# KrishnaswamyLab/MELD

Measured on AMD Instinct MI355X. Metric: cells/sec through MELD.fit_transform (kNN+Chebyshev), higher is better.
Workload: dtype f64

## Files before the change

include/meld_hip.h:

```cpp
#ifndef MELD_HIP_H
#define MELD_HIP_H

#include <stddef.h>
#include <stdint.h>

#ifdef __cplusplus
extern "C" {
#endif

#define MELD_OK 0
#define MELD_ERR_INVALID (-1)
#define MELD_ERR_UNSUPPORTED (-2)
#define MELD_ERR_HIP (-3)

typedef void* meld_stream_t;

int meld_abi_version(void);
const char* meld_last_error(void);
int meld_device_count(void);


int meld_knn_padded_dim(int d);
int meld_knn_tile_refs(void);
int meld_knn_block_queries(void);
// ... 50 lines not shown
                      int nprod, void* temp, void* lb2, meld_stream_t stream);
int meld_knn16_prepare_cross(const double* X, int64_t n_refs, int64_t n_total, int d, const double* mean, int64_t q_begin,
                             int64_t q_count, void* Rt16, void* Q16, float* Qn, float* norm2, float* norm2_max,
                             float* scale_info, meld_stream_t stream);
int meld_knn16_prepare_rows(const double* X, int64_t N, int d, const double* mean, const float* scale_info,
                            int64_t q_begin, const int32_t* rows, int64_t n_rows, void* Q16, float* Qn,
                            meld_stream_t stream);
int meld_knn16_research_thresholds(const int32_t* rows, int64_t n_rows, int64_t q_begin, const int32_t* cand_cnt,
                                   const float* cand_d2, int cap, int ksel, const float* norm2, const float* norm2_max,
                                   double err_coef, double err_lin, double err3, const float* scale_info, float* thr,
                                   meld_stream_t stream);
int meld_knn16_seed_thresholds_mfma(const void* Q16, const float* Qn, const void* Rt16, const float* scale_info,
                                    const float* norm2_max, int64_t n_ref, int d, int64_t q_begin, int64_t q_count,
                                    int knn, double radius_factor, int nprod, int side_tiles, float* thr_init,
                                    meld_stream_t stream);
int meld_knn16_topk(const void* Q16, const float* Qn, const void* Rt16, const float* scale_info,
                    int64_t n_ref, int d, int64_t q_count, int ksel, int nprod, int n_slices, const void* lb2,
                    const float* norm2_max, int64_t q_begin, const float* thr_init, int knn, double radius_factor,
                    int32_t* cand_idx, float* cand_d2, int32_t* cand_cnt, float* cand_thr,
                    uint64_t* tiles_done ,
                    const int32_t* block_order ,
                    meld_stream_t stream);
int meld_knn16_block_work(const void* lb2, const float* thr_seed, int64_t n_ref, int d, int64_t q_count, int nprod,
                          const float* norm2_max, const float* scale_info, int32_t* work, meld_stream_t stream);
int meld_knn16_step_lists(const void* lb2, const float* thr_seed, int64_t n_ref, int d, int64_t q_count, int nprod,
                          const float* norm2_max, const float* scale_info, int64_t q_begin, uint32_t* list,
                          int64_t list_stride, int32_t* cnt, meld_stream_t stream);
size_t meld_knn16_list_scratch_bytes(int64_t n_ref);
int meld_knn16_step_lists_direct(const double* X, int64_t N, int d, const double* mean, const float* scale_info, const float* norm2_max,
                                 const void* Rt16, const float* thr_seed, const float* q_norm2, int nprod, void* temp, void* scratch,
                                 uint32_t* list, int64_t list_stride, int32_t* cnt, meld_stream_t stream);
int meld_knn16_step_lists_direct_lead(const double* X, int64_t N, int d, const double* mean, const float* scale_info, const float* norm2_max,
                                 const void* Rt16, const float* thr_seed, const float* q_norm2, int nprod, void* temp, void* scratch,
                                 uint32_t* list, int64_t list_stride, int32_t* cnt, int lead_only, meld_stream_t stream);
int meld_knn16_step_lists_direct_spheres(const double* X, int64_t N, int d, const double* mean, const float* scale_info, const float* norm2_max,
                                 const void* Rt16, const float* thr_seed, const float* q_norm2, int nprod, void* temp, void* scratch,
                                 uint32_t* list, int64_t list_stride, int32_t* cnt, int lead_only, meld_stream_t stream);
int meld_knn16_topk_listed(const void* Q16, const float* Qn, const void* Rt16, const float* scale_info, int64_t n_ref, int d,
                           int64_t q_count, int ksel, const uint32_t* step_list, const int32_t* step_cnt, int64_t list_stride,
                           const float* norm2_max, int64_t q_begin, const float* thr_init, int knn, double radius_factor,
                           int32_t* cand_idx, float* cand_d2, int32_t* cand_cnt, float* cand_thr, uint64_t* tiles_done,
                           const int32_t* block_order, int n_slices , meld_stream_t stream);
int meld_knn16_topk_listed_partial(const void* Q16, const float* Qn, const void* Rt16, const float* scale_info, int64_t n_ref,
                                   int d, int64_t q_count, int ksel, const uint32_t* step_list, const int32_t* step_cnt,
                                   int64_t list_stride, const float* norm2_max, int64_t q_begin, const float* thr_init, int knn,
                                   double radius_factor, int32_t* cand_idx, float* cand_d2, int32_t* cand_cnt, float* cand_thr,
                                   uint64_t* tiles_done, const int32_t* block_order, int n_slices, int partial_test,
                                   meld_stream_t stream);
int meld_knn16_partial_filter(const void* Q16, const float* Qn, const void* Rt16, const float* scale_info, const float* norm2_max, int d,
                              int64_t q_count, const float* thr_init, uint32_t* step_list, const int32_t* step_cnt, int64_t list_stride,
                              int32_t* cnt_out, uint64_t* tested, const int32_t* block_order , meld_stream_t stream);
int meld_knn16_resident_blocks(int d, int nprod);
int meld_knn16_max_slices(int ksel);
int meld_knn16_merge_slices(const int32_t* s_idx, const float* s_d2, const int32_t* s_cnt, int64_t q_count,
                            int ksel, int n_slices, int32_t* out_idx, float* out_d2, int32_t* out_cnt,
                            meld_stream_t stream);


int meld_knn_refine(const double* X, int64_t N, int d, int64_t q_begin, int64_t q_count,
                    const int32_t* cand_idx, const float* cand_d2, const int32_t* cand_cnt,
                    const float* cand_thr ,
                    int ksel, int cap , int knn, double decay, double thresh,
                    const float* norm2_max, double err_coef,
                    const float* norm2 , double err_coef_lin, double* bw,
                    double* cand_val, int32_t* keep_cnt, int32_t* flag_rows, int32_t* n_flag,
                    const int32_t* rows, int out_cap, int32_t* cand_idx_out,
                    double bw_scale ,
                    const double* bw_fixed ,
                    int max_rank ,
                    meld_stream_t stream);

int meld_knn_radius_exact(const double* X, int64_t N, int d, int64_t q_begin, const int32_t* flag_rows,
                          int32_t n_flag, const double* bw, int knn, double decay, double thresh,
                          int mode, int32_t* fb_cnt, const int64_t* fb_off, int32_t* fb_cursor,
                          int32_t* fb_col, double* fb_val, int32_t* err_flag,
                          double bw_scale ,
                          meld_stream_t stream);
int meld_knn_pair_distances(const double* X, int d, const int64_t* rows, const int64_t* cand, int64_t n, int kk, double* out,
                            meld_stream_t stream);

#define MELD_METRIC_L1 1
#define MELD_METRIC_LINF 2
int meld_metric_tile_rows(void);
int meld_metric_tile_boxes(const double* X, int64_t N, int d, double* box_lo, double* box_hi, meld_stream_t stream);
int meld_metric_topk(const double* X, int64_t N, int d, int metric, int ksel, const double* box_lo, const double* box_hi, int prune,
                     double* heap_d, int32_t* heap_i, int32_t* cand_idx, double* cand_d, int32_t* cand_cnt,
                     unsigned long long* tiles_done, meld_stream_t stream);
int meld_metric_refine(const int32_t* cand_idx, const double* cand_d, const int32_t* cand_cnt, int64_t N, int ksel, int knn,
                       double decay, double thresh, double* bw, double* cand_val, int32_t* keep_cnt, int32_t* flag_rows,
                       int32_t* n_flag, meld_stream_t stream);
int meld_metric_radius(const double* X, int64_t N, int d, int metric, const int32_t* flag_rows, int32_t n_flag, const double* bw,
                       double decay, double thresh, int mode, int32_t* fb_cnt, const int64_t* fb_off, int32_t* fb_cursor,
                       int32_t* fb_col, double* fb_val, meld_stream_t stream);


size_t meld_scan_temp_bytes(int64_t n);
int meld_exclusive_scan_i32_i64(const int32_t* in, int64_t* out, int64_t n, void* temp, size_t temp_bytes,
                                meld_stream_t stream);

int meld_coo_emit(int64_t q_begin, int64_t q_count, const int32_t* cand_idx, const double* cand_val,
                  const int32_t* cand_cnt, int ksel, int cap, const int64_t* keep_off, const int32_t* flag_rows,
                  int32_t n_flag, const int64_t* fb_off, const int32_t* fb_col, const double* fb_val,
                  int64_t fb_base, int64_t M, uint64_t* keys, double* vals, meld_stream_t stream);

size_t meld_sort_temp_bytes(int64_t n);
int meld_sort_pairs_u64_f64(const uint64_t* keys_in, uint64_t* keys_out, const double* vals_in,
// ... 166 lines not shown
```

meld_amd/_lib.py:

```python
from __future__ import annotations

from ._options import is_set, opt

import ctypes as C
import os

_HERE = os.path.dirname(os.path.abspath(__file__))
LIB_NAME = "libmeld_hip.so"
LIB_PATH = os.path.join(_HERE, LIB_NAME)

_i32, _i64, _f64, _sz, _ptr = C.c_int, C.c_int64, C.c_double, C.c_size_t, C.c_void_p

SIGNATURES = {
    "meld_abi_version": (_i32, []),
    "meld_last_error": (C.c_char_p, []),
    "meld_device_count": (_i32, []),
    "meld_knn_padded_dim": (_i32, [_i32]),
    "meld_knn_tile_refs": (_i32, []),
    "meld_knn_block_queries": (_i32, []),
    "meld_knn_row_capacity": (_i32, [_i32]),
    "meld_col_sums_f64": (_i32, [_ptr, _i64, _i32, _ptr, _ptr]),
    "meld_col_stats_temp_bytes": (_sz, [_i32]),
    "meld_col_stats_f64": (_i32, [_ptr, _i64, _i32, _ptr, _ptr, _ptr, _ptr, _sz, _ptr]),
    "meld_knn_prepare_refs": (_i32, [_ptr, _i64, _i32, _ptr, _i32, _ptr, _ptr, _ptr, _ptr]),
    "meld_knn_prepare_queries": (_i32, [_ptr, _i64, _i32, _ptr, _i32, _i64, _i64, _ptr, _ptr]),
    "meld_knn_topk": (_i32, [_ptr, _ptr, _i64, _i32, _i64, _i32, _ptr, _ptr, _ptr, _ptr]),
    "meld_knn_refine": (
        _i32,
        [_ptr, _i64, _i32, _i64, _i64, _ptr, _ptr, _ptr, _ptr, _i32, _i32, _i32, _f64, _f64, _ptr, _f64, _ptr, _f64, _ptr, _ptr, _ptr,
         _ptr, _ptr, _ptr, _i32, _ptr, _f64, _ptr, _i32, _ptr],
    ),
    "meld_knn_error_coef": (_f64, [_i32]),
    "meld_knn16_kblocks": (_i32, [_i32]),
    "meld_knn16_tile_refs": (_i32, []),
    "meld_knn16_split_dims": (_i32, [_i32]),
    "meld_knn16_block_queries": (_i32, []),
    "meld_knn16_row_capacity": (_i32, [_i32]),
    "meld_knn16_error_coef": (_f64, [_i32, _i32]),
    "meld_knn16_error_coef_const": (_f64, [_i32, _i32]),
    "meld_knn16_error_coef_lin": (_f64, [_i32]),
    "meld_knn16_resident_blocks": (_i32, [_i32, _i32]),
    "meld_knn16_tile_bytes": (_sz, [_i32]),
    "meld_knn16_query_bytes": (_sz, [_i32]),
    "meld_knn16_prepare": (_i32, [_ptr, _i64, _i32, _ptr, _i64, _i64, _ptr, _ptr, _ptr, _ptr, _ptr, _ptr, _ptr]),
    "meld_knn16_prepare_scaled": (_i32, [_ptr, _i64, _i32, _ptr, _ptr, _ptr, _i64, _i64, _ptr, _ptr, _ptr, _ptr, _ptr, _ptr, _ptr]),
    "meld_knn16_prepare_cross": (_i32, [_ptr, _i64, _i64, _i32, _ptr, _i64, _i64, _ptr, _ptr, _ptr, _ptr, _ptr, _ptr, _ptr]),
    "meld_knn16_prepare_rows": (_i32, [_ptr, _i64, _i32, _ptr, _ptr, _i64, _ptr, _i64, _ptr, _ptr, _ptr]),
    "meld_knn16_research_thresholds": (_i32, [_ptr, _i64, _i64, _ptr, _ptr, _i32, _i32, _ptr, _ptr, _f64, _f64, _f64, _ptr, _ptr, _ptr]),
    "meld_knn16_bounds_bytes": (_sz, [_i64, _i64]),
    "meld_knn16_bounds_temp_bytes": (_sz, [_i64, _i32, _i64]),
    "meld_knn16_bounds": (_i32, [_ptr, _i64, _i32, _ptr, _ptr, _ptr, _ptr, _i64, _i64, _ptr, _ptr, _i32, _ptr, _ptr, _ptr]),
    "meld_knn16_bounds_from_spheres": (_i32, [_ptr, _i64, _i32, _ptr, _ptr, _ptr, _ptr, _i64, _i64, _ptr, _ptr, _i32, _ptr, _ptr, _ptr]),
    "meld_knn16_tile_spheres": (_i32, [_ptr, _i64, _i32, _ptr, _ptr, _ptr, _i64, _i64, _ptr]),
    "meld_knn16_sphere_layout": (_i32, [_i64, _i32, _ptr, _ptr]),
    "meld_knn16_topk": (_i32, [_ptr, _ptr, _ptr, _ptr, _i64, _i32, _i64, _i32, _i32, _i32, _ptr, _ptr, _i64, _ptr, _i32, _f64, _ptr, _ptr, _ptr, _ptr, _ptr, _ptr, _ptr]),
    "meld_knn16_block_work": (_i32, [_ptr, _ptr, _i64, _i32, _i64, _i32, _ptr, _ptr, _ptr, _ptr]),
    "meld_knn16_step_lists": (_i32, [_ptr, _ptr, _i64, _i32, _i64, _i32, _ptr, _ptr, _i64, _ptr, _i64, _ptr, _ptr]),
    "meld_knn16_list_scratch_bytes": (_sz, [_i64]),
    "meld_knn16_step_lists_direct": (_i32, [_ptr, _i64, _i32, _ptr, _ptr, _ptr, _ptr, _ptr, _ptr, _i32, _ptr, _ptr, _ptr, _i64, _ptr, _ptr]),
    "meld_knn16_prepare_fused": (_i32, [_ptr, _i64, _i32, _ptr, _ptr, _ptr, _ptr, _ptr, _ptr, _ptr, _ptr, _ptr, _ptr, _ptr]),
    "meld_knn16_step_lists_direct_spheres": (_i32, [_ptr, _i64, _i32, _ptr, _ptr, _ptr, _ptr, _ptr, _ptr, _i32, _ptr, _ptr, _ptr, _i64, _ptr, _i32, _ptr]),
    "meld_knn16_step_lists_direct_lead": (_i32, [_ptr, _i64, _i32, _ptr, _ptr, _ptr, _ptr, _ptr, _ptr, _i32, _ptr, _ptr, _ptr, _i64, _ptr, _i32, _ptr]),
    "meld_knn16_topk_listed": (_i32, [_ptr, _ptr, _ptr, _ptr, _i64, _i32, _i64, _i32, _ptr, _ptr, _i64, _ptr, _i64, _ptr, _i32, _f64, _ptr, _ptr, _ptr, _ptr, _ptr, _ptr, _i32, _ptr]),
    "meld_knn16_topk_listed_partial": (_i32, [_ptr, _ptr, _ptr, _ptr, _i64, _i32, _i64, _i32, _ptr, _ptr, _i64, _ptr, _i64, _ptr, _i32, _f64, _ptr, _ptr, _ptr, _ptr, _ptr, _ptr, _i32, _i32, _ptr]),
    "meld_knn16_partial_filter": (_i32, [_ptr, _ptr, _ptr, _ptr, _ptr, _i32, _i64, _ptr, _ptr, _ptr, _i64, _ptr, _ptr, _ptr, _ptr]),
    "meld_knn16_seed_thresholds_mfma": (_i32, [_ptr, _ptr, _ptr, _ptr, _ptr, _i64, _i32, _i64, _i64, _i32, _f64, _i32, _i32, _ptr, _ptr]),
    "meld_knn16_max_slices": (_i32, [_i32]),
    "meld_knn16_merge_slices": (_i32, [_ptr, _ptr, _ptr, _i64, _i32, _i32, _ptr, _ptr, _ptr, _ptr]),
    "meld_knn_radius_exact": (
        _i32,
        [_ptr, _i64, _i32, _i64, _ptr, _i32, _ptr, _i32, _f64, _f64, _i32, _ptr, _ptr, _ptr, _ptr, _ptr, _ptr, _f64, _ptr],
    ),
    "meld_knn_pair_distances": (_i32, [_ptr, _i32, _ptr, _ptr, _i64, _i32, _ptr, _ptr]),
    "meld_metric_tile_rows": (_i32, []),
    "meld_metric_tile_boxes": (_i32, [_ptr, _i64, _i32, _ptr, _ptr, _ptr]),
    "meld_metric_topk": (_i32, [_ptr, _i64, _i32, _i32, _i32, _ptr, _ptr, _i32, _ptr, _ptr, _ptr, _ptr, _ptr, _ptr, _ptr]),
    "meld_metric_refine": (_i32, [_ptr, _ptr, _ptr, _i64, _i32, _i32, _f64, _f64, _ptr, _ptr, _ptr, _ptr, _ptr, _ptr]),
    "meld_metric_radius": (_i32, [_ptr, _i64, _i32, _i32, _ptr, _i32, _ptr, _f64, _f64, _i32, _ptr, _ptr, _ptr, _ptr, _ptr, _ptr]),
    "meld_scan_temp_bytes": (_sz, [_i64]),
    "meld_exclusive_scan_i32_i64": (_i32, [_ptr, _ptr, _i64, _ptr, _sz, _ptr]),
    "meld_coo_emit": (
        _i32,
        [_i64, _i64, _ptr, _ptr, _ptr, _i32, _i32, _ptr, _ptr, _i32, _ptr, _ptr, _ptr, _i64, _i64, _ptr, _ptr, _ptr],
    ),
    "meld_sort_temp_bytes": (_sz, [_i64]),
    "meld_sort_pairs_u64_f64": (_i32, [_ptr, _ptr, _ptr, _ptr, _i64, _i32, _ptr, _sz, _ptr]),
    "meld_merge_temp_bytes": (_sz, [_i64]),
    "meld_coo_merge": (_i32, [_ptr, _ptr, _i64, _ptr, _ptr, _ptr, _ptr, _sz, _ptr]),
    "meld_csr_from_keys": (_i32, [_ptr, _i64, _i64, _i64, _ptr, _ptr, _ptr]),
    "meld_csr_seg_length": (_i32, []),
    "meld_csr_spmm_f64": (_i32, [_ptr, _ptr, _ptr, _i32, _i64, _ptr, _ptr, _i64, _ptr, _ptr, _i64, _ptr, _ptr, _i64, _i32, _ptr, _i64, _ptr]),
    "meld_csr_transpose_keys": (_i32, [_ptr, _ptr, _ptr, _i32, _i64, _ptr, _ptr, _ptr]),
    "meld_csr_rows_to_dense_f64": (_i32, [_ptr, _ptr, _ptr, _i32, _i64, _i64, _i64, _ptr, _i64, _ptr]),
    "meld_csr_bucket_slots": (_i32, []),
    "meld_coo_scatter_rows": (_i32, [_ptr, _ptr, _i64, _i64, _i64, _ptr, _ptr, _ptr, _ptr]),
    "meld_coo_emit_scatter": (_i32, [_i64, _ptr, _ptr, _i32, _i32, _ptr, _ptr, _i32, _ptr, _ptr, _ptr, _i64, _ptr, _ptr, _ptr, _ptr]),
    "meld_coo_partition_remote": (_i32, [_ptr, _ptr, _i64, _i64, _i32, _i32, _i64, _ptr, _ptr, _ptr]),
    "meld_csr_rows_sort_merge": (_i32, [_ptr, _i64, _ptr, _ptr, _ptr, _ptr, _i32, _f64, _ptr]),
    "meld_csr_compact_rows": (_i32, [_ptr, _i64, _ptr, _ptr, _ptr, _ptr, _ptr]),
    "meld_csr_rows_sort_merge_sums": (_i32, [_ptr, _i64, _ptr, _ptr, _ptr, _ptr, _i32, _f64, _f64, _ptr, _ptr]),
    "meld_csr_compact_rows_anisotropy": (_i32, [_ptr, _i64, _ptr, _ptr, _ptr, _ptr, _ptr, _f64, _ptr, _ptr]),
    "meld_csr_compact_rows_sums": (_i32, [_ptr, _i64, _ptr, _ptr, _ptr, _ptr, _f64, _ptr, _ptr]),
    "meld_csr_row_sums": (_i32, [_ptr, _ptr, _i64, _f64, _ptr, _ptr]),
    "meld_csr_anisotropy": (_i32, [_ptr, _ptr, _ptr, _i64, _ptr, _i64, _f64, _ptr]),
    "meld_csr_anisotropy_degrees": (_i32, [_ptr, _ptr, _ptr, _i64, _ptr, _i64, _f64, _ptr, _ptr]),
    "meld_spmm_dot_slots": (_i32, []),
    "meld_cheby_step": (
        _i32,
        [_ptr, _ptr, _ptr, _ptr, _i64, _i64, _i32, _ptr, _i64, _ptr, _ptr, _ptr, _f64, _f64, _f64, _f64, _ptr, _ptr],
    ),
    "meld_lanczos_steps": (_i32, [_ptr, _ptr, _ptr, _ptr, _i64, _i64, _ptr, _ptr, _ptr, _ptr, _ptr, _ptr, _i32, _i32, _ptr, _ptr]),
    "meld_lanczos_spmv": (_i32, [_ptr, _ptr, _ptr, _ptr, _i64, _i64, _ptr, _i64, _ptr, _ptr, _ptr, _ptr, _ptr]),
    "meld_lanczos_alpha": (_i32, [_ptr, _ptr, _ptr, _ptr, _i32, _ptr]),
    "meld_lanczos_axpy": (_i32, [_ptr, _ptr, _i64, _ptr, _ptr, _ptr]),
    "meld_lanczos_beta": (_i32, [_ptr, _ptr, _ptr, _ptr, _i32, _ptr]),
    "meld_lanczos_fold": (_i32, [_ptr, _ptr, _ptr, _ptr, _i32, _ptr]),
    "meld_lanczos_axpy3": (_i32, [_ptr, _ptr, _ptr, _i64, _ptr, _ptr, _ptr]),
    "meld_pt_geometry": (_i32, [_ptr, _ptr, _ptr, _ptr]),
    "meld_pt_num_blocks": (_i32, [_i64]),
    "meld_pt_seg_len": (_i64, [_i32]),
# ... 87 lines not shown
```

meld_amd/csrc/knn16.hip:

```cpp
#include "common.hpp"

#include <hip/hip_fp16.h>

#include <algorithm>

namespace meld {

constexpr int K16_TS = 64;
constexpr int K16_BQ = 256;
constexpr int K16_THREADS = 256;
constexpr int K16_NWAVE = K16_THREADS / 64;
constexpr int K16_SLACK = 128;
constexpr int K16_CAPMAX = 256;
constexpr int K16_BOUNDS_THREADS = 1024;
constexpr int K16_SLOTS = K16_CAPMAX / 64;
constexpr int K16_DMAX = 16 * 9 - 3;

constexpr int K16_SPLIT_DA = 13;
__host__ __device__ inline void k16_slot(int c, int d, int dA, int* coord, int* piece) {
  *coord = -1;
  *piece = -1;
  if (dA == 0) {
    if (c < d) *coord = c;
    else if (c < d + 3) *piece = 3 + (c - d);
    return;
  }
  const int nb = d - dA;
  if (c < dA) *coord = c;
  else if (c < dA + 3) *piece = c - dA;
  else if (c < 16) return;
  else if (c < 16 + nb) *coord = dA + (c - 16);
  else if (c < 16 + nb + 3) *piece = 3 + (c - 16 - nb);
}

typedef float f32x16 __attribute__((ext_vector_type(16)));
typedef _Float16 f16x8 __attribute__((ext_vector_type(8)));

__device__ __forceinline__ float min3f(float a, float b, float c) { return __builtin_fminf(__builtin_fminf(a, b), c); }
__device__ __forceinline__ float min16(const f32x16& v) {
  const float a = min3f(v[0], v[1], v[2]);
  const float b = min3f(v[3], v[4], v[5]);
  const float c = min3f(v[6], v[7], v[8]);
  const float d = min3f(v[9], v[10], v[11]);
  const float e = min3f(v[12], v[13], v[14]);
  return __builtin_fminf(min3f(a, b, v[15]), min3f(c, d, e));
}

__device__ __forceinline__ unsigned ordered_bits(float f) {
  const unsigned b = __float_as_uint(f);
  return (b & 0x80000000u) ? ~b : (b | 0x80000000u);
}

__device__ __forceinline__ float ld_sc1_f(const float* p) {
  return __hip_atomic_load(p, __ATOMIC_RELAXED, __HIP_MEMORY_SCOPE_AGENT);
}
__device__ __forceinline__ int ld_sc1_i(const int* p) {
  return __hip_atomic_load(p, __ATOMIC_RELAXED, __HIP_MEMORY_SCOPE_AGENT);
}

#define K16_COLD_REGION_END() __builtin_amdgcn_s_waitcnt(0x0F70)

__device__ __forceinline__ bool knn16_row_slot(int p, int n0, int n1, int half, int* q) {
  if (p < half) {
    *q = p;
    return p < n0;
  }
  *q = n0 + (p - half);
  return (p - half) < n1;
}
__device__ __forceinline__ int knn16_split_pos(int pos, int m0, int half) { return pos < m0 ? pos : half + (pos - m0); }

__device__ __forceinline__ float from_ordered_bits(unsigned k) {
  return __uint_as_float((k & 0x80000000u) ? (k & 0x7fffffffu) : ~k);
}

__device__ float knn16_squeeze_row(int n0, int n1, int half, int ksel, int knn1, float rf2, float err, float nq_row,
                                   float* __restrict__ d2row, int* __restrict__ idxrow, int lane, int* n0_out,
                                   int* n1_out, float* r_out) {
  asm volatile("s_waitcnt vmcnt(0)" ::: "memory");
  float d[K16_SLOTS];
  int ix[K16_SLOTS];
  unsigned key[K16_SLOTS];
  bool valid[K16_SLOTS];
#pragma unroll
  for (int e = 0; e < K16_SLOTS; ++e) {
    const int p = lane + 64 * e;
    int q;
    valid[e] = p < 2 * half && knn16_row_slot(p, n0, n1, half, &q);
    if (valid[e]) {
      d[e] = ld_sc1_f(d2row + p);
      ix[e] = ld_sc1_i(idxrow + p);
      key[e] = ordered_bits(d[e]);
    } else {
      d[e] = INFINITY;
      ix[e] = 0x7fffffff;
      key[e] = 0xffffffffu;
    }
  }
  unsigned T = 0;
#pragma unroll 1
  for (int bit = 31; bit >= 0; --bit) {
    const unsigned trial = T | (1u << bit);
    int c = 0;
#pragma unroll
    for (int e = 0; e < K16_SLOTS; ++e) c += __popcll(__ballot(key[e] < trial));
    if (c < ksel) T = trial;
  }
  float R = INFINITY;
  if (knn1 > 0 && n0 + n1 >= knn1) {
    unsigned A = 0;
#pragma unroll 1
    for (int bit = 31; bit >= 0; --bit) {
      const unsigned trial = A | (1u << bit);
      int c = 0;
#pragma unroll
      for (int e = 0; e < K16_SLOTS; ++e) c += __popcll(__ballot(key[e] < trial));
      if (c < knn1) A = trial;
    }
    R = (rf2 * ((from_ordered_bits(A) + nq_row) + err) + err) * 1.00001f + 1e-30f - nq_row;
  }
  *r_out = R;
  const unsigned Tc = min(T, ordered_bits(R));
  int total = 0;
#pragma unroll
  for (int e = 0; e < K16_SLOTS; ++e) total += __popcll(__ballot(valid[e] && key[e] <= Tc));
  const int m0 = (total + 1) >> 1;
  int base = 0;
  float thr = INFINITY;
#pragma unroll
  for (int e = 0; e < K16_SLOTS; ++e) {
    const bool keep = valid[e] && key[e] <= Tc;
    const unsigned long long b = __ballot(keep);
    if (keep) {
      const int dst = knn16_split_pos(base + __popcll(b & ((1ull << lane) - 1ull)), m0, half);
      d2row[dst] = d[e];
      idxrow[dst] = ix[e];
    }
    base += __popcll(b);
    const unsigned long long bt = __ballot(valid[e] && key[e] == T);
    if (bt) thr = __shfl(d[e], __ffsll((long long)bt) - 1, 64);
  }
  *n0_out = m0;
  *n1_out = total - m0;
  return thr;
}

__device__ void knn16_rank_row(int n0, int n1, int half, int ksel, float out_scale, float add, int split_m0,
                               float* __restrict__ d2row, int* __restrict__ idxrow, float* sd, int* si, int lane) {
  asm volatile("s_waitcnt vmcnt(0)" ::: "memory");
  const int n = n0 + n1;
  float d[K16_SLOTS];
  int ix[K16_SLOTS];
  bool valid[K16_SLOTS];
#pragma unroll
  for (int e = 0; e < K16_SLOTS; ++e) {
    const int p = lane + 64 * e;
    int q = 0;
    valid[e] = p < 2 * half && knn16_row_slot(p, n0, n1, half, &q);
    if (valid[e]) {
      d[e] = ld_sc1_f(d2row + p);
      ix[e] = ld_sc1_i(idxrow + p);
      sd[q] = d[e];
      si[q] = ix[e];
    } else {
      d[e] = INFINITY;
      ix[e] = 0x7fffffff;
    }
  }
  asm volatile("s_waitcnt lgkmcnt(0)" ::: "memory");
  int rk[K16_SLOTS];
#pragma unroll
  for (int q = 0; q < K16_SLOTS; ++q) rk[q] = 0;
  for (int e = 0; e < n; ++e) {
    const float de = sd[e];
    const int ie = si[e];
#pragma unroll
    for (int q = 0; q < K16_SLOTS; ++q) rk[q] += (de < d[q] || (de == d[q] && ie < ix[q])) ? 1 : 0;
  }
#pragma unroll
  for (int q = 0; q < K16_SLOTS; ++q) {
    if (valid[q] && rk[q] < ksel) {
      const int dst = split_m0 < 0 ? rk[q] : knn16_split_pos(rk[q], split_m0, half);
      d2row[dst] = (d[q] + add) * out_scale;
      idxrow[dst] = ix[q];
    }
  }
  asm volatile("s_waitcnt lgkmcnt(0)" ::: "memory");
}

__device__ __forceinline__ int k16_scan_tile(int s, int t0, int n_scan, int two_sided) {
  int off = s;
  if (two_sided && s >= K16_BQ / K16_TS) {
    const int j = s - K16_BQ / K16_TS;
    off = (j & 1) ? -1 - (j >> 1) : K16_BQ / K16_TS + (j >> 1);
  }
  const int t = t0 + off;
  return t >= n_scan ? t - n_scan : (t < 0 ? t + n_scan : t);
}

struct K16Args {
  const _Float16* Q16;
  const float* Qn;
  const _Float16* Rt16;
  const float* scale_info;
  int n_ref, n_tiles, ksel, cap;
  const __half* lb2;
  const float* norm2_max;
  float err_coef;
  int tile_origin, batch_every, batch_slack, two_sided;
  unsigned long long* stats;
  const float* thr_init;
  int knn1;
  float rf2, err_c, err_l;
  int* cand_idx;
  float* cand_d2;
  int* cand_cnt;
  float* cand_thr;
  unsigned long long* tiles_done;
  const int* block_order;
  const unsigned* step_list;
  const int* step_cnt;
  long long list_stride;
  int ee_hi;
  int planes_used;
  int count_go;
};
#define K16_COLD(FIELD) \
  (((const volatile K16Args __attribute__((address_space(4)))*)__builtin_amdgcn_kernarg_segment_ptr())->FIELD)
// ... 194 lines not shown
#pragma unroll
  for (int g = 0; g < 2; ++g) {
#pragma unroll
    for (int kb = 0; kb < KB; ++kb) {
      asm volatile("" : "+v"(bhi[g][kb]));
      if (NPROD == 3) asm volatile("" : "+v"(blo[g][kb]));
    }
    asm volatile("" : "+v"(thrp[g]));
  }

  f32x16 accA0, accA1, accB0, accB1;
#pragma unroll
  for (int r = 0; r < 16; ++r) accB0[r] = accB1[r] = INFINITY;
  int refB = 0;

  auto mfma_block = [&](const _Float16* tile, int sub, f32x16& c0, f32x16& c1) __attribute__((always_inline)) {
#pragma unroll
    for (int r = 0; r < 16; ++r) c0[r] = c1[r] = 0.0f;
    const f16x8* a8 = reinterpret_cast<const f16x8*>(tile) + sub * 32 + jq;
#pragma unroll
    for (int kb = 0; kb < KB; ++kb) {
      const f16x8 ahi = NPROD == 3 ? a8[((kb * 2 + h) * 2 + 0) * K16_TS] : a8[(kb * 2 + h) * K16_TS];
      c0 = __builtin_amdgcn_mfma_f32_32x32x16_f16(ahi, bhi[0][kb], c0, 0, 0, 0);
      c1 = __builtin_amdgcn_mfma_f32_32x32x16_f16(ahi, bhi[1][kb], c1, 0, 0, 0);
      if (NPROD == 3) {
        const f16x8 alo = a8[((kb * 2 + h) * 2 + 1) * K16_TS];
        c0 = __builtin_amdgcn_mfma_f32_32x32x16_f16(ahi, blo[0][kb], c0, 0, 0, 0);
        c1 = __builtin_amdgcn_mfma_f32_32x32x16_f16(ahi, blo[1][kb], c1, 0, 0, 0);
        c0 = __builtin_amdgcn_mfma_f32_32x32x16_f16(alo, bhi[0][kb], c0, 0, 0, 0);
        c1 = __builtin_amdgcn_mfma_f32_32x32x16_f16(alo, bhi[1][kb], c1, 0, 0, 0);
      }
    }
  };
  auto vote = [&](const f32x16& c0, const f32x16& c1, float& m0, float& m1) __attribute__((always_inline)) {
    m0 = min16(c0);
    m1 = min16(c1);
  };
  auto squeeze = [&](int g, int j) __attribute__((always_inline)) {
    const int cg = g ? cnt[1] : cnt[0];
    const int n0 = __shfl(cg, j, 64), n1 = __shfl(cg, j + 32, 64);
    const size_t ro = (size_t)(g * 32 + j) * cap;
    int m0, m1;
    float rcut = INFINITY, err = 0.0f;
    const int knn1 = K16_COLD(knn1);
    const float nq_row = wave_qn[g * 32 + j];
    if (knn1 > 0) {
      const float* sinfo = K16_COLD(scale_info);
      const float nmax_s = K16_COLD(norm2_max)[0] * sinfo[0] * sinfo[0];
      err = (K16_COLD(err_c) * nmax_s + K16_COLD(err_l) * sqrtf(nq_row * nmax_s)) * 1.001f;
    }
    float nt = knn16_squeeze_row(n0, n1, half, ksel, knn1, K16_COLD(rf2), err, nq_row, wave_d2 + ro, wave_idx + ro, lane, &m0, &m1, &rcut);
    if (m0 > half - 32) {
      knn16_rank_row(m0, m1, half, ksel, 1.0f, 0.0f, (min(m0 + m1, ksel) + 1) >> 1, wave_d2 + ro, wave_idx + ro, lds_sd[wave],
                     lds_si[wave], lane);
      const int tot = min(m0 + m1, ksel);
      m0 = (tot + 1) >> 1;
      m1 = tot - m0;
      asm volatile("s_waitcnt vmcnt(0)" ::: "memory");
      nt = ld_sc1_f(wave_d2 + ro + knn16_split_pos(tot - 1, m0, half));
    }
    if (jq == j) {
      const int mine = h ? m1 : m0;
      if (g) cnt[1] = mine; else cnt[0] = mine;
      const float t_list = (n0 + n1 >= ksel) ? nt : INFINITY;
      thrp[g] = fminf(thrp[g], fminf(t_list, rcut));
    }
    asm volatile("" : "+v"(thrp[0]), "+v"(thrp[1]), "+v"(cnt[0]), "+v"(cnt[1]));
  };
  auto refresh_wmax = [&]() __attribute__((always_inline)) {
    if (my_lb == nullptr) return;
    float w = fmaxf(thrp[0] + wave_qn[jq], thrp[1] + wave_qn[32 + jq]);
#pragma unroll
    for (int off = 32; off > 0; off >>= 1) w = fmaxf(w, __shfl_xor(w, off, 64));
    wmax = w;
  };
  auto select = [&](const f32x16& c0, const f32x16& c1, float m0, float m1, int ref_base) __attribute__((always_inline)) {
    unsigned long long need = 0;
    if (STATS) ++st_slow;
#pragma unroll
    for (int g = 0; g < 2; ++g) {
      const f32x16 acc = g ? c1 : c0;
      if (!__any((g ? m1 : m0) < thrp[g])) continue;
      const unsigned rowoff4 = (unsigned)((g * 32 + jq) * cap + h * half) * 4u;
      auto append = [&](int r) __attribute__((always_inline)) {
        const float v = acc[r];
        if (v < thrp[g]) {
          const unsigned off4 = rowoff4 + 4u * (unsigned)(g ? cnt[1]++ : cnt[0]++);
          if (STATS) ++st_app;
          *reinterpret_cast<float*>(reinterpret_cast<char*>(wave_d2) + off4) = v;
          *reinterpret_cast<int*>(reinterpret_cast<char*>(wave_idx) + off4) = ref_base + (r & 3) + 8 * (r >> 2);
        }
      };
#pragma unroll
      for (int t = 0; t < 5; ++t) {
        if (__any(min3f(acc[3 * t], acc[3 * t + 1], acc[3 * t + 2]) < thrp[g])) {
          append(3 * t);
          append(3 * t + 1);
          append(3 * t + 2);
        }
      }
      if (__any(acc[15] < thrp[g])) append(15);
      const unsigned long long full = __ballot((g ? cnt[1] : cnt[0]) > half - 16);
      need |= ((full | (full >> 32)) & 0xffffffffull) << (32 * g);
    }
    if (__builtin_expect(need != 0, 0)) {
      while (need) {
        const int j = __ffsll((long long)need) - 1;
// ... 175 lines not shown
          todo &= todo - 1;
          squeeze(j >> 5, j & 31);
          if (STATS) ++st_sq;
        }
        refresh_wmax();
        K16_COLD_REGION_END();
      }
    }

    bool live_nn = true;
    int s_nn, t_nn;
    if constexpr (LIST) {
      s_nn = min(s_next + 1, n_scan);
      t_nn = s_nn < n_scan ? (int)(e_pref & 0xFFFFFFu) : t_next;
      live_nn = entry_live(e_pref);
      e_pref = e_far;
    } else {
      s_nn = s_next < n_scan ? next_step(s_next, par, &live_nn) : n_scan;
      t_nn = s_nn < n_scan ? tile_of(s_nn) : t_next;
    }

    if (s_nn < n_scan) {
      K16_LOAD(__builtin_amdgcn_readfirstlane(t_nn), wr_b);
      tm_lap(tm_tail);
      K16_STAGED_BUT_LAST();
    } else {
      tm_lap(tm_tail);
      K16_STAGED();
    }
    tm_lap(tm_dma);
    if (my_lb) {
      my_live = __ballot(win_lb <= wmax + prune_margin);
      if (lane == 0) lds_wlive[par ^ 1][wave] = my_live;
    }
    tm_lap(tm_tail);
    K16_TILE_BARRIER();
    tm_lap(tm_bar);
    s_cur = s_next;
    t_cur = t_next;
    live_cur = live_next;
    s_next = s_nn;
    t_next = t_nn;
    live_next = live_nn;
    par ^= 1;
    ++it;
    const unsigned free_b = rd_b;
    rd_b = nx_b;
    nx_b = wr_b;
    wr_b = free_b;
  };
  tm_mark = tm_now();
  if constexpr (PAIR) {
    constexpr unsigned PB = 2u * (unsigned)TILE_LDS_BYTES;
    const int n_pairs = (n_scan + 1) >> 1;
    unsigned c0 = list_entry(0), c1 = list_entry(1), x0 = list_entry(2), x1 = list_entry(3);
    if (n_scan > 0) K16_LOAD(__builtin_amdgcn_readfirstlane((int)(c0 & 0xFFFFFFu)), 0u);
    if (n_scan > 1) K16_LOAD(__builtin_amdgcn_readfirstlane((int)(c1 & 0xFFFFFFu)), (unsigned)TILE_LDS_BYTES);
    K16_STAGED();
    K16_TILE_BARRIER();
    for (int p = 0; p < n_pairs; ++p) {
      const unsigned buf = (p & 1) ? PB : 0u, other = PB - buf;
      const unsigned f0 = list_entry(2 * p + 4), f1 = list_entry(2 * p + 5);
      if (2 * p + 2 < n_scan) K16_LOAD(__builtin_amdgcn_readfirstlane((int)(x0 & 0xFFFFFFu)), other);
      if (2 * p + 3 < n_scan) K16_LOAD(__builtin_amdgcn_readfirstlane((int)(x1 & 0xFFFFFFu)), other + (unsigned)TILE_LDS_BYTES);
      tm_lap(tm_tail);
      const char* ring = reinterpret_cast<const char*>(lds_ring);
      const bool live0 = entry_live(c0), live1 = 2 * p + 1 < n_scan && entry_live(c1);
      if (live0) ee_tile(reinterpret_cast<const _Float16*>(ring + buf), (int)(c0 & 0xFFFFFFu));
      if (live1) ee_tile(reinterpret_cast<const _Float16*>(ring + buf + TILE_LDS_BYTES), (int)(c1 & 0xFFFFFFu));
      if (live0 || live1) tm_lap(tm_seg); else tm_lap(tm_idle);
      if (batch_every > 0 && (p & (batch_every / 2 - 1)) == batch_every / 2 - 1) {
        const int limit = ksel + K16_COLD(batch_slack);
        unsigned long long todo = 0;
#pragma unroll
        for (int g = 0; g < 2; ++g) {
          const int cg = g ? cnt[1] : cnt[0];
          const int tot = cg + __shfl_xor(cg, 32, 64);
          todo |= (__ballot(tot > limit) & 0xffffffffull) << (32 * g);
        }
        while (todo) {
          const int j = __ffsll((long long)todo) - 1;
          todo &= todo - 1;
          squeeze(j >> 5, j & 31);
          if (STATS) ++st_sq;
        }
      }
      tm_lap(tm_tail);
      K16_STAGED();
      tm_lap(tm_dma);
      K16_TILE_BARRIER();
      tm_lap(tm_bar);
      c0 = x0;
      c1 = x1;
      x0 = f0;
      x1 = f1;
      ++it;
    }
  }
  while (!PAIR && s_cur < n_scan) scan_step();
  if (pend) segment(nullptr, 0, accA0, accA1, accB0, accB1, refB, false, true);
  {
    unsigned long long* tiles_done = K16_COLD(tiles_done);
    if (tiles_done && lane == 0) {
      atomicAdd(tiles_done, (unsigned long long)n_done);
      if (EE && K16_COLD(count_go)) atomicAdd(tiles_done + 1, (unsigned long long)st_go);
    }
  }

  unsigned long long* stats = STATS ? K16_COLD(stats) : nullptr;
  if (STATS && stats) {
    unsigned a = st_app;
#pragma unroll
    for (int off = 32; off > 0; off >>= 1) a += __shfl_xor(a, off, 64);
    if (lane == 0) {
      atomicAdd(stats + 0, (unsigned long long)(2 * n_done));
      atomicAdd(stats + 1, (unsigned long long)st_slow);
      atomicAdd(stats + 2, (unsigned long long)a);
      atomicAdd(stats + 3, (unsigned long long)st_sq);
      const int it_tiles = PAIR ? n_scan : it;
      if (wave == 0) atomicAdd(stats + 4, (unsigned long long)it_tiles);
      atomicAdd(stats + 5, (unsigned long long)tm_seg);
      atomicAdd(stats + 6, (unsigned long long)tm_sel);
      atomicAdd(stats + 7, (unsigned long long)tm_tail);
      atomicAdd(stats + 8, (unsigned long long)tm_dma);
      atomicAdd(stats + 9, (unsigned long long)tm_bar);
      atomicAdd(stats + 10, (unsigned long long)tm_idle);
      atomicAdd(stats + 11, (unsigned long long)it_tiles);
      if (EE) atomicAdd(stats + 12, (unsigned long long)st_go);
    }
  }
  const float out_scale = K16_COLD(scale_info)[1];
  float* cand_thr = K16_COLD(cand_thr);
  int* cand_cnt = K16_COLD(cand_cnt);
  if (cand_thr && h == 0) {
    cand_thr[row_base + jq] = (thrp[0] + wave_qn[jq]) * out_scale;
    cand_thr[row_base + 32 + jq] = (thrp[1] + wave_qn[32 + jq]) * out_scale;
  }
  {
    const int o0 = __shfl_xor(cnt[0], 32, 64), o1 = __shfl_xor(cnt[1], 32, 64);
    if (h == 0) {
      cand_cnt[row_base + jq] = cnt[0] | (o0 << 16);
      cand_cnt[row_base + 32 + jq] = cnt[1] | (o1 << 16);
    }
  }
#undef K16_LOAD
#undef K16_DMA
#undef K16_STAGED
#undef K16_STAGED_BUT_LAST
#undef K16_TILE_BARRIER
#undef K16_ROUND_OK
}

template <int TPS, int WPE>
__global__ __launch_bounds__(256) __attribute__((amdgpu_waves_per_eu(WPE, WPE))) void knn16_partial_filter_kernel(const _Float16* __restrict__ Q16, const float* __restrict__ Qn,
                                                                   const _Float16* __restrict__ Rt16, const float* __restrict__ scale_info,
                                                                   const float* __restrict__ norm2_max, const float* __restrict__ thr_init,
                                                                   unsigned* step_list, const int* __restrict__ step_cnt, long long list_stride,
                                                                   int* __restrict__ cnt_out, unsigned long long* __restrict__ tested,
                                                                   const int* __restrict__ block_order, int KB, int ee_hi) {
  static_assert(TPS >= 2 && TPS <= 32 && (TPS & 1) == 0, "tiles per step");
  __shared__ __attribute__((aligned(16))) _Float16 ring[2][TPS][2 * K16_TS * 8];
  __shared__ unsigned wmask[2][4];
  const int tid = threadIdx.x, lane = tid & 63;
  const int wave = __builtin_amdgcn_readfirstlane(tid >> 6);
  const int jq = lane & 31, h = lane >> 5;
  const int bx = block_order ? __builtin_amdgcn_readfirstlane(block_order[blockIdx.x]) : (int)blockIdx.x;
  const int q_base = bx * K16_BQ + wave * 64;
  f16x8 b0[2];
  float tA[2];
  {
    const float s_ = scale_info[0];
    const float delta = 3.814697265625e-06f * (norm2_max[0] * s_ * s_) + 1e-30f;
#pragma unroll
    for (int g = 0; g < 2; ++g) {
      const int q = q_base + g * 32 + jq;
      const f16x8* qrow = reinterpret_cast<const f16x8*>(Q16 + (size_t)q * (size_t)(KB * 32));
      b0[g] = qrow[h * 2];
      float qb = 0.0f;
      for (int kb = 1; kb < KB; ++kb) {
        const f16x8 v8 = qrow[(kb * 2 + h) * 2];
#pragma unroll
        for (int e = 0; e < 8; ++e) {
          const float v = (16 * kb + 8 * h + e < ee_hi) ? (float)v8[e] : 0.0f;
          qb = fmaf(v, v, qb);
        }
      }
      qb += __shfl_xor(qb, 32, 64);
      tA[g] = (thr_init[q] - Qn[q]) + (qb * 1.0001f + delta);
    }
  }
  unsigned* const my_list_w = step_list + (size_t)bx * (size_t)list_stride;
  const int n = __builtin_amdgcn_readfirstlane(step_cnt[bx]);
  const int n_steps = (n + TPS - 1) / TPS;
  const size_t tile_bytes = (size_t)KB * 4096;
  const int plane_stride = 2048;
  const size_t src_base = reinterpret_cast<size_t>(Rt16);
  typedef __attribute__((address_space(3))) void* lds_ptr_t;
  typedef int i32x4 __attribute__((ext_vector_type(4)));
  const unsigned ring_base = (unsigned)(size_t)(lds_ptr_t)&ring[0][0][0];
  const int lane16 = lane * 16;
  auto load_entries = [&](int step) __attribute__((always_inline)) {
    const int idx = step * TPS + lane;
    return (lane < TPS && idx < n) ? my_list_w[idx] : 0u;
  };
  auto stage = [&](unsigned ev, int buf) __attribute__((always_inline)) {
#pragma unroll
    for (int u = 0; u < TPS / 2; ++u) {
      const int k = wave * (TPS / 2) + u;
      const unsigned e = (unsigned)__builtin_amdgcn_readlane((int)ev, k >> 1);
      if (e >> 24) {
        const size_t src = src_base + (size_t)(e & 0xFFFFFFu) * tile_bytes;
// ... 1647 lines not shown
}

extern "C" int meld_knn16_partial_filter(const void* Q16, const float* Qn, const void* Rt16, const float* scale_info, const float* norm2_max,
                                         int d, int64_t q_count, const float* thr_init, uint32_t* step_list, const int32_t* step_cnt,
                                         int64_t list_stride, int32_t* cnt_out, uint64_t* tested, const int32_t* block_order,
                                         meld_stream_t stream) {
  MELD_CHECK_ARG(Q16 && Qn && Rt16 && scale_info && norm2_max && thr_init && step_list && step_cnt && cnt_out && list_stride > 0 && q_count > 0,
                 "meld_knn16_partial_filter: null pointer or bad sizes");
  const int KB = meld_knn16_kblocks(d);
  if (KB < 0) return KB;
  const int dA = k16_dA(d, KB);
  MELD_CHECK_ARG(dA > 0 && KB >= 2, "meld_knn16_partial_filter: d = %d has no split operand layout", d);
  const unsigned n_blocks = (unsigned)ceil_div(q_count, K16_BQ);
  hipLaunchKernelGGL((knn16_partial_filter_kernel<8, 4>), dim3(n_blocks), dim3(256), 0, S(stream), reinterpret_cast<const _Float16*>(Q16), Qn,
                     reinterpret_cast<const _Float16*>(Rt16), scale_info, norm2_max, thr_init, step_list, step_cnt, (long long)list_stride, cnt_out,
                     reinterpret_cast<unsigned long long*>(tested), block_order, KB, 16 + d - dA);
  MELD_LAUNCH_CHECK("knn16_partial_filter_kernel");
  return MELD_OK;
}

extern "C" int meld_knn16_resident_blocks(int d, int nprod) {
  MELD_CHECK_ARG(nprod == 1 || nprod == 3, "meld_knn16_resident_blocks: nprod must be 1 or 3");
  const int KB = meld_knn16_kblocks(d);
  if (KB < 0) return KB;
  int per_cu = 0;
#define K16_OCC(KBV)                                                                                              \
  case KBV:                                                                                                       \
    if (nprod == 1) {                                                                                             \
      MELD_HIP_CALL(hipOccupancyMaxActiveBlocksPerMultiprocessor(&per_cu, knn16_topk_kernel<KBV, 0, 1>, K16_THREADS, 0)); \
    } else {                                                                                                      \
      MELD_HIP_CALL(hipOccupancyMaxActiveBlocksPerMultiprocessor(&per_cu, knn16_topk_kernel<KBV, 0, 3>, K16_THREADS, 0)); \
    }                                                                                                             \
    break;
  switch (KB) {
    K16_OCC(1)
    K16_OCC(2)
    K16_OCC(3)
    K16_OCC(4)
    K16_OCC(5)
    K16_OCC(6)
    K16_OCC(7)
    K16_OCC(8)
    K16_OCC(9)
    default:
      return MELD_ERR_UNSUPPORTED;
  }
#undef K16_OCC
  int dev = 0, cus = 0;
  MELD_HIP_CALL(hipGetDevice(&dev));
  MELD_HIP_CALL(hipDeviceGetAttribute(&cus, hipDeviceAttributeMultiprocessorCount, dev));
  return per_cu * cus;
}

extern "C" int meld_knn16_max_slices(int ksel) { return ksel < 1 ? MELD_ERR_INVALID : std::max(1, K16_MERGE_MAX / ksel); }

extern "C" int meld_knn16_merge_slices(const int32_t* s_idx, const float* s_d2, const int32_t* s_cnt, int64_t q_count,
                                       int ksel, int n_slices, int32_t* out_idx, float* out_d2, int32_t* out_cnt,
                                       meld_stream_t stream) {
  MELD_CHECK_ARG(s_idx && s_d2 && s_cnt && out_idx && out_d2 && out_cnt && q_count > 0, "meld_knn16_merge_slices: null");
  const int cap = meld_knn16_row_capacity(ksel);
  if (cap < 0) return cap;
  MELD_CHECK_ARG(n_slices >= 1 && n_slices * ksel <= K16_MERGE_MAX, "meld_knn16_merge_slices: too many slices");
  const int q_pad = (int)(ceil_div(q_count, K16_BQ) * K16_BQ);
  hipLaunchKernelGGL(knn16_merge_slices_kernel, dim3((unsigned)q_count), dim3(64), (size_t)n_slices * ksel * 8, S(stream), s_idx, s_d2,
                     s_cnt, (int)q_count, q_pad, ksel, cap, n_slices, out_idx, out_d2, out_cnt);
  MELD_LAUNCH_CHECK("knn16_merge_slices_kernel");
  return MELD_OK;
}
```

Baseline: 28.55 million.

## Replace per-pair tile barrier with LDS counter ring handshake in paired kNN scan

In the paired-tile scan loop, the workgroup-wide barrier after each tile pair is replaced by LDS-resident producer/consumer counters. Waves spin with s_sleep until the current buffer is marked ready, and the next tiles are prefetched early once all waves have released the other buffer. The aim is to let waves drift relative to each other instead of stalling at a barrier every step. It adds spin-wait overhead, a timeout counter with a host query function, and reserves the last LDS words of one wave's rank scratch, so the rank routine falls back to global reads beyond that limit. If the memory-ordering assumptions are wrong, this can race.

```diff
diff --git a/include/meld_hip.h b/include/meld_hip.h
--- a/include/meld_hip.h
+++ b/include/meld_hip.h
@@ -126,6 +126,7 @@
                               int32_t* cnt_out, uint64_t* tested, const int32_t* block_order , meld_stream_t stream);
 int meld_knn16_resident_blocks(int d, int nprod);
 int meld_knn16_max_slices(int ksel);
+int meld_knn16_ring_timeouts(void);
 int meld_knn16_merge_slices(const int32_t* s_idx, const float* s_d2, const int32_t* s_cnt, int64_t q_count,
                             int ksel, int n_slices, int32_t* out_idx, float* out_d2, int32_t* out_cnt,
                             meld_stream_t stream);
diff --git a/meld_amd/_lib.py b/meld_amd/_lib.py
--- a/meld_amd/_lib.py
+++ b/meld_amd/_lib.py
@@ -66,6 +66,7 @@
     "meld_knn16_partial_filter": (_i32, [_ptr, _ptr, _ptr, _ptr, _ptr, _i32, _i64, _ptr, _ptr, _ptr, _i64, _ptr, _ptr, _ptr, _ptr]),
     "meld_knn16_seed_thresholds_mfma": (_i32, [_ptr, _ptr, _ptr, _ptr, _ptr, _i64, _i32, _i64, _i64, _i32, _f64, _i32, _i32, _ptr, _ptr]),
     "meld_knn16_max_slices": (_i32, [_i32]),
+    "meld_knn16_ring_timeouts": (_i32, []),
     "meld_knn16_merge_slices": (_i32, [_ptr, _ptr, _ptr, _i64, _i32, _i32, _ptr, _ptr, _ptr, _ptr]),
     "meld_knn_radius_exact": (
         _i32,
diff --git a/meld_amd/csrc/knn16.hip b/meld_amd/csrc/knn16.hip
--- a/meld_amd/csrc/knn16.hip
+++ b/meld_amd/csrc/knn16.hip
@@ -14,6 +14,7 @@
 constexpr int K16_CAPMAX = 256;
 constexpr int K16_BOUNDS_THREADS = 1024;
 constexpr int K16_SLOTS = K16_CAPMAX / 64;
+constexpr int K16_RING_WORDS = 4;
 constexpr int K16_DMAX = 16 * 9 - 3;
 
 constexpr int K16_SPLIT_DA = 13;
@@ -57,6 +58,13 @@
 __device__ __forceinline__ int ld_sc1_i(const int* p) {
   return __hip_atomic_load(p, __ATOMIC_RELAXED, __HIP_MEMORY_SCOPE_AGENT);
 }
+
+__device__ __forceinline__ int k16_lds_peek(const int* p) {
+  return __builtin_amdgcn_readfirstlane(__hip_atomic_load(p, __ATOMIC_RELAXED, __HIP_MEMORY_SCOPE_WORKGROUP));
+}
+__device__ __forceinline__ void k16_lds_bump(int* p) { __hip_atomic_fetch_add(p, 1, __ATOMIC_RELAXED, __HIP_MEMORY_SCOPE_WORKGROUP); }
+constexpr int K16_SPIN_MAX = 1 << 22;
+__device__ unsigned int k16_ring_timeouts = 0;
 
 #define K16_COLD_REGION_END() __builtin_amdgcn_s_waitcnt(0x0F70)
 
@@ -146,7 +154,7 @@
 }
 
 __device__ void knn16_rank_row(int n0, int n1, int half, int ksel, float out_scale, float add, int split_m0,
-                               float* __restrict__ d2row, int* __restrict__ idxrow, float* sd, int* si, int lane) {
+                               float* __restrict__ d2row, int* __restrict__ idxrow, float* sd, int* si, int lane, int lim) {
   asm volatile("s_waitcnt vmcnt(0)" ::: "memory");
   const int n = n0 + n1;
   float d[K16_SLOTS];
@@ -160,8 +168,10 @@
     if (valid[e]) {
       d[e] = ld_sc1_f(d2row + p);
       ix[e] = ld_sc1_i(idxrow + p);
-      sd[q] = d[e];
-      si[q] = ix[e];
+      if (q < lim) {
+        sd[q] = d[e];
+        si[q] = ix[e];
+      }
     } else {
       d[e] = INFINITY;
       ix[e] = 0x7fffffff;
@@ -171,9 +181,16 @@
   int rk[K16_SLOTS];
 #pragma unroll
   for (int q = 0; q < K16_SLOTS; ++q) rk[q] = 0;
-  for (int e = 0; e < n; ++e) {
+  for (int e = 0; e < min(n, lim); ++e) {
     const float de = sd[e];
     const int ie = si[e];
+#pragma unroll
+    for (int q = 0; q < K16_SLOTS; ++q) rk[q] += (de < d[q] || (de == d[q] && ie < ix[q])) ? 1 : 0;
+  }
+  for (int e = lim; e < n; ++e) {
+    const int p = e < n0 ? e : half + (e - n0);
+    const float de = ld_sc1_f(d2row + p);
+    const int ie = ld_sc1_i(idxrow + p);
 #pragma unroll
     for (int q = 0; q < K16_SLOTS; ++q) rk[q] += (de < d[q] || (de == d[q] && ie < ix[q])) ? 1 : 0;
   }
@@ -474,7 +491,7 @@
     float nt = knn16_squeeze_row(n0, n1, half, ksel, knn1, K16_COLD(rf2), err, nq_row, wave_d2 + ro, wave_idx + ro, lane, &m0, &m1, &rcut);
     if (m0 > half - 32) {
       knn16_rank_row(m0, m1, half, ksel, 1.0f, 0.0f, (min(m0 + m1, ksel) + 1) >> 1, wave_d2 + ro, wave_idx + ro, lds_sd[wave],
-                     lds_si[wave], lane);
+                     lds_si[wave], lane, PAIR ? K16_CAPMAX - K16_RING_WORDS : K16_CAPMAX);
       const int tot = min(m0 + m1, ksel);
       m0 = (tot + 1) >> 1;
       m1 = tot - m0;
@@ -756,22 +773,50 @@
   tm_mark = tm_now();
   if constexpr (PAIR) {
     constexpr unsigned PB = 2u * (unsigned)TILE_LDS_BYTES;
+    int* const ring_cnt = &lds_si[K16_NWAVE - 1][K16_CAPMAX - K16_RING_WORDS];
+    auto ring_wait = [&](const int* c, int need) __attribute__((always_inline)) {
+      if (__builtin_expect(k16_lds_peek(c) < need, 0)) {
+        int rounds = 0;
+        do {
+          __builtin_amdgcn_s_sleep(1);
+          if (++rounds > K16_SPIN_MAX) {
+            if (lane == 0) atomicAdd(&k16_ring_timeouts, 1u);
+            break;
+          }
+        } while (k16_lds_peek(c) < need);
+      }
+      asm volatile("" ::: "memory");
+    };
     const int n_pairs = (n_scan + 1) >> 1;
     unsigned c0 = list_entry(0), c1 = list_entry(1), x0 = list_entry(2), x1 = list_entry(3);
+    if (tid < K16_RING_WORDS) ring_cnt[tid] = tid == 0 ? K16_NWAVE : 0;
     if (n_scan > 0) K16_LOAD(__builtin_amdgcn_readfirstlane((int)(c0 & 0xFFFFFFu)), 0u);
     if (n_scan > 1) K16_LOAD(__builtin_amdgcn_readfirstlane((int)(c1 & 0xFFFFFFu)), (unsigned)TILE_LDS_BYTES);
     K16_STAGED();
     K16_TILE_BARRIER();
     for (int p = 0; p < n_pairs; ++p) {
-      const unsigned buf = (p & 1) ? PB : 0u, other = PB - buf;
+      const int slot = p & 1;
+      const unsigned buf = slot ? PB : 0u, other = PB - buf;
       const unsigned f0 = list_entry(2 * p + 4), f1 = list_entry(2 * p + 5);
-      if (2 * p + 2 < n_scan) K16_LOAD(__builtin_amdgcn_readfirstlane((int)(x0 & 0xFFFFFFu)), other);
-      if (2 * p + 3 < n_scan) K16_LOAD(__builtin_amdgcn_readfirstlane((int)(x1 & 0xFFFFFFu)), other + (unsigned)TILE_LDS_BYTES);
+      const bool have_next = 2 * p + 2 < n_scan;
+      const int need_cur = K16_NWAVE * ((p >> 1) + 1);
+      const int need_free = K16_NWAVE * ((p + 1) >> 1);
+      bool requested = !have_next;
+      if (!requested && k16_lds_peek(&ring_cnt[2 + (slot ^ 1)]) >= need_free) {
+        asm volatile("" ::: "memory");
+        K16_LOAD(__builtin_amdgcn_readfirstlane((int)(x0 & 0xFFFFFFu)), other);
+        if (2 * p + 3 < n_scan) K16_LOAD(__builtin_amdgcn_readfirstlane((int)(x1 & 0xFFFFFFu)), other + (unsigned)TILE_LDS_BYTES);
+        requested = true;
+      }
       tm_lap(tm_tail);
+      ring_wait(&ring_cnt[slot], need_cur);
+      tm_lap(tm_bar);
       const char* ring = reinterpret_cast<const char*>(lds_ring);
       const bool live0 = entry_live(c0), live1 = 2 * p + 1 < n_scan && entry_live(c1);
       if (live0) ee_tile(reinterpret_cast<const _Float16*>(ring + buf), (int)(c0 & 0xFFFFFFu));
       if (live1) ee_tile(reinterpret_cast<const _Float16*>(ring + buf + TILE_LDS_BYTES), (int)(c1 & 0xFFFFFFu));
+      asm volatile("s_waitcnt lgkmcnt(0)" ::: "memory");
+      if (lane == 0) k16_lds_bump(&ring_cnt[2 + slot]);
       if (live0 || live1) tm_lap(tm_seg); else tm_lap(tm_idle);
       if (batch_every > 0 && (p & (batch_every / 2 - 1)) == batch_every / 2 - 1) {
         const int limit = ksel + K16_COLD(batch_slack);
@@ -790,10 +835,17 @@
         }
       }
       tm_lap(tm_tail);
-      K16_STAGED();
-      tm_lap(tm_dma);
-      K16_TILE_BARRIER();
-      tm_lap(tm_bar);
+      if (have_next) {
+        if (!requested) {
+          ring_wait(&ring_cnt[2 + (slot ^ 1)], need_free);
+          tm_lap(tm_bar);
+          K16_LOAD(__builtin_amdgcn_readfirstlane((int)(x0 & 0xFFFFFFu)), other);
+          if (2 * p + 3 < n_scan) K16_LOAD(__builtin_amdgcn_readfirstlane((int)(x1 & 0xFFFFFFu)), other + (unsigned)TILE_LDS_BYTES);
+        }
+        K16_STAGED();
+        tm_lap(tm_dma);
+        if (lane == 0) k16_lds_bump(&ring_cnt[slot ^ 1]);
+      }
       c0 = x0;
       c1 = x1;
       x0 = f0;
@@ -859,8 +911,8 @@
 __global__ __launch_bounds__(256) __attribute__((amdgpu_waves_per_eu(WPE, WPE))) void knn16_partial_filter_kernel(const _Float16* __restrict__ Q16, const float* __restrict__ Qn,
                                                                    const _Float16* __restrict__ Rt16, const float* __restrict__ scale_info,
                                                                    const float* __restrict__ norm2_max, const float* __restrict__ thr_init,
-                                                                   unsigned* step_list, const int* __restrict__ step_cnt, long long list_stride,
-                                                                   int* __restrict__ cnt_out, unsigned long long* __restrict__ tested,
+                                                                   unsigned* step_list, const int* step_cnt, long long list_stride,
+                                                                   int* cnt_out, unsigned long long* __restrict__ tested,
                                                                    const int* __restrict__ block_order, int KB, int ee_hi) {
   static_assert(TPS >= 2 && TPS <= 32 && (TPS & 1) == 0, "tiles per step");
   __shared__ __attribute__((aligned(16))) _Float16 ring[2][TPS][2 * K16_TS * 8];
@@ -2614,6 +2666,12 @@
   return per_cu * cus;
 }
 
+extern "C" int meld_knn16_ring_timeouts() {
+  unsigned int n = 0;
+  MELD_HIP_CALL(hipMemcpyFromSymbol(&n, HIP_SYMBOL(k16_ring_timeouts), sizeof(n)));
+  return (int)std::min(n, 0x7fffffffu);
+}
+
 extern "C" int meld_knn16_max_slices(int ksel) { return ksel < 1 ? MELD_ERR_INVALID : std::max(1, K16_MERGE_MAX / ksel); }
 
 extern "C" int meld_knn16_merge_slices(const int32_t* s_idx, const float* s_d2, const int32_t* s_cnt, int64_t q_count,
```

Result: slower. 27.74 million (-2.8%).
